# seungjunlee96/lightning-generative-models

Hardware: AMD Instinct MI355X
Metric: training images/sec (DDPM UNet 32x32, bs=128) (higher is better)
Workload: dtype f32

## Files before the change

lightning-generative-models_amd/csrc/winograd.hip:

```cpp
#include <stdlib.h>

#include <type_traits>

#include "lgm_common.h"

int lgm_splitk_reduce_launch(const float* ws, long ws_stride, int splits, const float* bias, const float* res,
                             long res_pitch, float* out, long out_pitch, long M, int N, hipStream_t s);

static void* lgm_wino_debug_buffer = nullptr;
static int lgm_wino_debug_mode = 0;
extern "C" int lgm_wino_set_debug_buffer(void* buf, int mode) {
  lgm_wino_debug_buffer = buf;
  lgm_wino_debug_mode = mode;
  return LGM_OK;
}

#ifndef LGM_STORE_AUX
#define LGM_STORE_AUX 0
#endif

namespace lgmwino {
typedef unsigned int u32x4 __attribute__((ext_vector_type(4)));
typedef float f32x2 __attribute__((ext_vector_type(2)));

// ... 1304 lines not shown
    w[k] = (double)gs[k]->B * gs[k]->H * gs[k]->W * gs[k]->Nw * gs[k]->Cw;
    tot += w[k];
    mn[k] = 2L * (gs[k]->Nw / 64) * (gs[k]->Cw / 32);
  }
  for (int k = 0; k < n; ++k) {
    long b = (long)((double)lgm_cu_budget() * w[k] / tot + (n == 2 && k == 0 ? 0.5 : 0.0));
    if (b < mn[k]) b = mn[k];
    budget[k] = b;
    left -= b;
  }
  int big = 0;
  for (int k = 1; k < n; ++k)
    if (budget[k] - mn[k] > budget[big] - mn[big]) big = k;
  budget[big] += left;
  if (budget[big] < mn[big]) budget[big] = mn[big];
}

static bool wgradn_supported(int n, const LgmConvGeom* const* gs) {
  using namespace lgmwino;
  if (n < 2 || n > 8) return false;
  if (n > 4) {
    for (int k = 0; k < n; ++k)
      if (!gs[k]) return false;
    return wgradn_use4(n, gs);
  }
  int G0 = 0;
  long need = 0;
  static const bool alone4 = getenv("LGM_W4W_ALONE") ? atoi(getenv("LGM_W4W_ALONE")) != 0 : true;
  if (alone4 && !wgradn_use4(n, gs)) {
    bool all4 = true;
    for (int k = 0; k < n; ++k) all4 = all4 && gs[k] && lgm_wino4_wgrad_use(gs[k]);
    if (all4) return false;
  }
  for (int k = 0; k < n; ++k) {
    if (!gs[k] || !lgm_wino_wgrad_supported(gs[k])) return false;
    int G, ipc;
    wgrad_class(gs[k]->H, gs[k]->W, &G, &ipc);
    if (k == 0) G0 = G;
    else if (G != G0) return false;
    need += 2L * (gs[k]->Nw / 64) * (gs[k]->Cw / 64);
  }
  return need <= lgm_cu_budget();
}

static void wgradn_budgets(int n, const LgmConvGeom* const* gs, long* budget) {
  double w[4], tot = 0;
  long mn[4], left = lgm_cu_budget();
  for (int k = 0; k < n; ++k) {
    w[k] = (double)gs[k]->B * gs[k]->H * gs[k]->W * gs[k]->Nw * gs[k]->Cw;
    tot += w[k];
    mn[k] = 2L * (gs[k]->Nw / 64) * (gs[k]->Cw / 64);
  }
  for (int k = 0; k < n; ++k) {
    long b = (long)((double)lgm_cu_budget() * w[k] / tot);
    if (b < mn[k]) b = mn[k];
    budget[k] = b;
    left -= b;
  }
  int big = 0;
  for (int k = 1; k < n; ++k)
    if (budget[k] - mn[k] > budget[big] - mn[big]) big = k;
  budget[big] += left;
  if (budget[big] < mn[big]) budget[big] = mn[big];
}

extern "C" int64_t lgm_conv3x3_wino_wgradn_supported(int n, const LgmConvGeom* const* geoms) {
// ... 280 lines not shown
```

lightning-generative-models_amd/csrc/winograd4.hip:

```cpp
#include <atomic>
#include <stdlib.h>

#include <type_traits>

#include "lgm_common.h"

int lgm_splitk_reduce_launch(const float* ws, long ws_stride, int splits, const float* bias, const float* res,
                             long res_pitch, float* out, long out_pitch, long M, int N, hipStream_t s);

static void* lgm_wino4_debug_buffer = nullptr;
static int lgm_wino4_debug_exp = 0;
static int lgm_wino4_debug_slots = 0;
static int lgm_wino4_debug_next = 0;
extern "C" int lgm_wino4_set_debug_buffer(void* buf, int exp) {
  lgm_wino4_debug_buffer = buf;
  lgm_wino4_debug_exp = exp & 0xffff;
  lgm_wino4_debug_slots = exp >> 16;
  lgm_wino4_debug_next = 0;
  return LGM_OK;
}

#ifndef LGM_WINO4_PFU
#define LGM_WINO4_PFU 1
#endif

namespace lgmwino4 {
typedef unsigned int u32x4 __attribute__((ext_vector_type(4)));
typedef float f32x2 __attribute__((ext_vector_type(2)));

constexpr int KC = 8;
constexpr int NXI = 36;
constexpr int VBUF = NXI * 256;
constexpr int MBUF = NXI * 32 * 32;

template <int CLS>
struct Geo;
template <>
struct Geo<0> {
  static constexpr int NI = 1, TTH = 4, TTW = 8, PH = 18, PW = 34, RS = 34, IMG = PH * RS, PLANE = 641;
};
template <>
struct Geo<1> {
  static constexpr int NI = 2, TTH = 4, TTW = 4, PH = 18, PW = 18, RS = 20, IMG = PH * RS, PLANE = 737;
};
template <>
struct Geo<2> {
  static constexpr int NI = 8, TTH = 2, TTW = 2, PH = 10, PW = 10, RS = 10, IMG = 112, PLANE = 897;
};

struct Args {
  const float* a;
  const float* u;
  const float* bias;
  const float* res;
  float* out;
  long a_pitch, res_pitch, out_pitch;
  int B, H, W;
  int C;
  int N;
  int tb_h, tb_w, tiles_n, nbg;
  int splits, pps, units;
  int tn_slowest;
  int xcd_ranges;
  float* ws;
  long ws_stride;
  long long* dbg;
  float* stats;
};

__device__ __forceinline__ f32x4 add4(const f32x4 a, const f32x4 b) { return a + b; }
__device__ __forceinline__ f32x4 sub4(const f32x4 a, const f32x4 b) {
  f32x2 lo, hi;
  asm("v_pk_add_f32 %0, %1, %2 neg_lo:[0,1] neg_hi:[0,1]"
      : "=v"(lo)
      : "v"(__builtin_shufflevector(a, a, 0, 1)), "v"(__builtin_shufflevector(b, b, 0, 1)));
  asm("v_pk_add_f32 %0, %1, %2 neg_lo:[0,1] neg_hi:[0,1]"
      : "=v"(hi)
      : "v"(__builtin_shufflevector(a, a, 2, 3)), "v"(__builtin_shufflevector(b, b, 2, 3)));
  return __builtin_shufflevector(lo, hi, 0, 1, 2, 3);
}
__device__ __forceinline__ f32x4 fma4(const float c, const f32x4 a, const f32x4 b) {
  return __builtin_elementwise_fma(f32x4{c, c, c, c}, a, b);
}
__device__ __forceinline__ f32x2 fma2(const float c, const f32x2 a, const f32x2 b) {
  return __builtin_elementwise_fma(f32x2{c, c}, a, b);
}

template <int CLS, bool DBG = false, int EXP = 0, bool STATS = false>
__global__ __launch_bounds__(512, 2) void wino4_conv_kernel(const Args p) {
  using GE = Geo<CLS>;
  constexpr bool PFU = LGM_WINO4_PFU != 0;
  int nstamp = 0;
  auto stamp = [&]() {
    if (DBG) {
      if (threadIdx.x == 0 && nstamp < 30) p.dbg[blockIdx.x * 32 + 1 + nstamp] = (long long)__builtin_amdgcn_s_memtime();
      ++nstamp;
    }
  };
  stamp();
  const long long rt_entry = DBG ? (long long)__builtin_amdgcn_s_memrealtime() : 0;
  constexpr int NI = GE::NI, PH = GE::PH, PW = GE::PW, RS = GE::RS, IMG = GE::IMG, PLANE = GE::PLANE;
  constexpr int RBUF = 8 * PLANE;
  constexpr int NPIX = NI * PH * PW;
  constexpr int NJ = (2 * NPIX + 511) / 512;
  extern __shared__ __align__(16) float smem[];
  float* const Rb = smem;
  float* const Vb = smem + 2 * RBUF;
  float* const Mb = smem;
  const int tid = threadIdx.x;
  const int lane = tid & 63;
  const int wid = __builtin_amdgcn_readfirstlane(tid >> 6);
  const int lr = lane & 31, lh = lane >> 5;

  int L = (p.xcd_ranges && (gridDim.x & 7) == 0) ? (int)((blockIdx.x & 7) * (gridDim.x >> 3) + (blockIdx.x >> 3)) : (int)blockIdx.x;
  int tn, split, twi, thi, bg;
  if (p.tn_slowest) {
    twi = L % p.tb_w;
    L /= p.tb_w;
    thi = L % p.tb_h;
    L /= p.tb_h;
    bg = L % p.nbg;
    L /= p.nbg;
    split = L % p.splits;
    tn = L / p.splits;
  } else {
    tn = L % p.tiles_n;
    L /= p.tiles_n;
    split = L % p.splits;
    L /= p.splits;
    twi = L % p.tb_w;
    L /= p.tb_w;
    thi = L % p.tb_h;
    bg = L / p.tb_h;
  }
  const int n0 = tn * 64;
  const int h0 = thi * (4 * GE::TTH), w0 = twi * (4 * GE::TTW), b0 = bg * NI;
  const int ncc = p.C / KC;
  const int cc0 = split * p.pps;
  const int cc1 = min(ncc, cc0 + p.pps);
  const int nph = cc1 - cc0;

  const unsigned nrec_a = (unsigned)((long)p.B * p.H * p.W * p.a_pitch * 4);
  __amdgpu_buffer_rsrc_t rsrc_a;
  {
    const unsigned long long ab = reinterpret_cast<unsigned long long>(p.a);
    const unsigned lo = __builtin_amdgcn_readfirstlane((unsigned)ab);
    const unsigned hi = __builtin_amdgcn_readfirstlane((unsigned)(ab >> 32));
    rsrc_a = __builtin_amdgcn_make_buffer_rsrc(reinterpret_cast<void*>(((unsigned long long)hi << 32) | lo), 0,
                                               __builtin_amdgcn_readfirstlane(nrec_a), 0x00020000);
  }
  unsigned goff[NJ], plds[NJ];
#pragma unroll
  for (int j = 0; j < NJ; ++j) {
    const int s = tid + 512 * j;
    const int pix = s >> 1, q = s & 1;
    unsigned g = nrec_a, l = (unsigned)(q * 4 * PLANE + NI * IMG);
    if (pix < NPIX) {
      const int img = pix / (PH * PW);
      const int rem = pix - img * (PH * PW);
      const int py = rem / PW, px = rem - py * PW;
      const int gy = h0 - 1 + py, gx = w0 - 1 + px;
      l = (unsigned)(q * 4 * PLANE + img * IMG + py * RS + px);
      if (gy >= 0 && gy < p.H && gx >= 0 && gx < p.W)
        g = (unsigned)((((long)(b0 + img) * p.H + gy) * p.W + gx) * p.a_pitch + q * 4) * 4u;
    }
    goff[j] = g;
    plds[j] = l;
  }
  u32x4 rp[NJ];
  auto fetch1 = [&](int j, int ph) -> u32x4 {
    const unsigned soff = (unsigned)((cc0 + ph) * (KC * 4));
    return __builtin_amdgcn_raw_buffer_load_b128(rsrc_a, ph < nph ? goff[j] : nrec_a, soff, 0);
  };
  auto commit_r = [&](float* rbuf, int j, const u32x4 r) {
    float* d = rbuf + plds[j];
    const f32x4 f = __builtin_bit_cast(f32x4, r);
    d[0] = f[0];
    d[PLANE] = f[1];
    d[2 * PLANE] = f[2];
    d[3 * PLANE] = f[3];
  };
  u32x4 rq0[NJ], rq1[NJ];
#pragma unroll
  for (int j = 0; j < NJ; ++j) rq0[j] = fetch1(j, 0);
#pragma unroll
  for (int j = 0; j < NJ; ++j) rq1[j] = fetch1(j, 1);
#pragma unroll
  for (int j = 0; j < NJ; ++j) rp[j] = fetch1(j, 2);

  int t_tile, t_img, t_ty, t_tx;
  const int half = wid >> 2;
  const int tk = (lane & 3) + 4 * (lane >> 5);
  if (CLS == 0) {
    t_img = 0;
    t_ty = wid & 3;
    t_tx = (lane >> 2) & 7;
    t_tile = t_ty * 8 + t_tx;
  } else if (CLS == 1) {
    t_img = (wid >> 1) & 1;
    t_ty = 2 * (wid & 1) + ((lane >> 4) & 1);
    t_tx = (lane >> 2) & 3;
    t_tile = t_img * 16 + t_ty * 4 + t_tx;
  } else {
    t_img = 2 * (wid & 3) + ((lane >> 4) & 1);
    t_ty = (lane >> 3) & 1;
    t_tx = (lane >> 2) & 1;
    t_tile = t_img * 4 + t_ty * 2 + t_tx;
  }
  const int trd = tk * PLANE + t_img * IMG + 4 * t_ty * RS + 4 * t_tx;
  const int vwr = (tk >> 2) * 128 + t_tile * 4 + (tk & 3) + half * (18 * 256);

  const int xg = wid & 3, ch = wid >> 2;
  const int vrd = xg * (9 * 256) + lh * 128 + lr * 4;
  __amdgpu_buffer_rsrc_t rsrc_u;
  {
    const unsigned long long ub = reinterpret_cast<unsigned long long>(p.u);
    const unsigned lo = __builtin_amdgcn_readfirstlane((unsigned)ub);
    const unsigned hi = __builtin_amdgcn_readfirstlane((unsigned)(ub >> 32));
    rsrc_u = __builtin_amdgcn_make_buffer_rsrc(reinterpret_cast<void*>(((unsigned long long)hi << 32) | lo), 0,
                                               __builtin_amdgcn_readfirstlane((unsigned)((long)p.N * p.C * NXI * 4)),
                                               0x00020000);
  }
  const unsigned ulane = (unsigned)((ch * 64 + lane) * 16);
  const unsigned ubase = (unsigned)((tn * ncc + cc0) * NXI + xg * 9) * 2048u;
  unsigned pf = 0;
  if (PFU) {
    const unsigned ubytes = min((unsigned)nph * (NXI * 2048u), 2u << 20);
    const unsigned nx = gridDim.x >> 3;
    const unsigned spatial = (unsigned)(p.nbg * p.tb_h * p.tb_w);
    const unsigned grp = p.tn_slowest ? 1u : (unsigned)(p.tiles_n * p.splits);
    const unsigned share = p.tn_slowest ? ((unsigned)blockIdx.x >> 3) % spatial : ((unsigned)blockIdx.x >> 3) / grp;
    const unsigned nshare = p.tn_slowest ? min(nx, spatial) : nx / grp;
    const unsigned off = (share * 512u + (unsigned)tid) * 128u;
    if (p.xcd_ranges && (gridDim.x & 7) == 0 && off < ubytes && nshare * 512u * 128u >= ubytes)
      pf = __builtin_amdgcn_raw_buffer_load_b32(rsrc_u, off, (unsigned)((tn * ncc + cc0) * NXI) * 2048u, 0);
  }
  auto load_u = [&](int ph, int e) -> f32x4 {
    const unsigned soff = ubase + (unsigned)(ph * NXI + e) * 2048u;
    u32x4 v = __builtin_amdgcn_raw_buffer_load_b128(rsrc_u, ulane, soff, 0);
    return __builtin_bit_cast(f32x4, v);
  };

  auto body = [&](auto half_c) {
    constexpr int HALF = decltype(half_c)::value;
    f32x16 acc[9];
#pragma unroll
    for (int e = 0; e < 9; ++e)
#pragma unroll
      for (int r = 0; r < 16; ++r) acc[e][r] = 0.f;
    f32x2 T[3][3];
    int roff0 = trd, roff1 = RBUF + trd;
    asm volatile("" : "+v"(roff0));
    asm volatile("" : "+v"(roff1));
    auto stage1 = [&](int nxt, int cp) {
      const float* r = smem + (nxt ? roff1 : roff0);
      f32x2 d[6];
#pragma unroll
      for (int rr = 0; rr < 6; ++rr)
        if (rr != (HALF ? 0 : 5)) d[rr] = f32x2{r[rr * RS + 2 * cp], r[rr * RS + 2 * cp + 1]};
      if (HALF == 0) {
        T[0][cp] = fma2(4.f, d[0], fma2(-5.f, d[2], d[4]));
        const f32x2 a = fma2(-4.f, d[2], d[4]), b = fma2(-4.f, d[1], d[3]);
        T[1][cp] = a + b;
        T[2][cp] = a - b;
      } else {
        const f32x2 c = d[4] - d[2], f = d[3] - d[1];
        T[0][cp] = fma2(2.f, f, c);
        T[1][cp] = fma2(-2.f, f, c);
        T[2][cp] = fma2(4.f, d[1], fma2(-5.f, d[3], d[5]));
      }
    };
    auto stage2 = [&](float* vbuf, int i, int part) {
      float* v = vbuf + vwr + i * (6 * 256);
      const float t0 = T[i][0][0], t1 = T[i][0][1], t2 = T[i][1][0], t3 = T[i][1][1], t4 = T[i][2][0], t5 = T[i][2][1];
      if (part == 0) {
        const float a = __builtin_fmaf(-4.f, t2, t4), b = __builtin_fmaf(-4.f, t1, t3);
        v[0 * 256] = __builtin_fmaf(4.f, t0, __builtin_fmaf(-5.f, t2, t4));
        v[1 * 256] = a + b;
        v[2 * 256] = a - b;
      } else {
        const float c = t4 - t2, f = t3 - t1;
        v[3 * 256] = __builtin_fmaf(2.f, f, c);
        v[4 * 256] = __builtin_fmaf(-2.f, f, c);
        v[5 * 256] = __builtin_fmaf(4.f, t1, __builtin_fmaf(-5.f, t3, t5));
      }
    };

    stamp();
    f32x4 uq[3];
#pragma unroll
    for (int e = 0; e < 3; ++e) uq[e] = load_u(0, e);
    if (DBG) __builtin_amdgcn_sched_barrier(0);
    stamp();
#pragma unroll
    for (int j = 0; j < NJ; ++j) commit_r(Rb, j, rq0[j]);
#pragma unroll
    for (int j = 0; j < NJ; ++j) commit_r(Rb + RBUF, j, rq1[j]);
    if (DBG) __builtin_amdgcn_sched_barrier(0);
    stamp();
    __syncthreads();
    if (PFU) asm volatile("" ::"v"(pf));
    stamp();
#pragma unroll
    for (int cp = 0; cp < 3; ++cp) stage1(0, cp);
#pragma unroll
    for (int i = 0; i < 3; ++i) {
      stage2(Vb, i, 0);
// ... 19 lines not shown
        for (int s = 0; s < 4; ++s) acc[e] = __builtin_amdgcn_mfma_f32_32x32x2f32(uf[s], vf[s], acc[e], 0, 0, 0);
        if (!(EXP & 4)) uq[e % 3] = (e + 3 < 9) ? load_u(ph, e + 3) : load_u(ph + 1, e + 3 - 9);
        if (!(EXP & 1)) {
          if (e < 3) stage1(cur ^ 1, e);
          else stage2(vnxt, (e - 3) >> 1, (e - 3) & 1);
        }
        if (e >= 9 - NJ && !(EXP & 2)) {
          commit_r(rcur, e - (9 - NJ), rp[e - (9 - NJ)]);
          rp[e - (9 - NJ)] = fetch1(e - (9 - NJ), ph + 3);
        }
        vf = vfn;
        __builtin_amdgcn_sched_barrier(0);
      }
      static_assert(NJ >= 1 && NJ <= 4, "the commit is dealt out over the last NJ steps");
      __syncthreads();
      stamp();
    };
    for (int ph = 0; ph < nph; ph += 2) {
      phase(ph, std::integral_constant<int, 0>{});
      if (ph + 1 < nph) phase(ph + 1, std::integral_constant<int, 1>{});
    }

    const int th = tid & 255;
    const int eq = th & 3, et = (th >> 2) & 31, rpair = __builtin_amdgcn_readfirstlane(th >> 7);
    int e_img, e_ty, e_tx;
    if (CLS == 0) {
      e_img = 0;
      e_ty = et >> 3;
      e_tx = et & 7;
    } else if (CLS == 1) {
      e_img = et >> 4;
      e_ty = (et >> 2) & 3;
      e_tx = et & 3;
    } else {
      e_img = et >> 2;
      e_ty = (et >> 1) & 1;
      e_tx = et & 1;
    }
    const long opix = ((long)(b0 + e_img) * p.H + h0 + 4 * e_ty) * p.W + w0 + 4 * e_tx;
    const bool partial = p.splits > 1;
    const int ncol0 = n0 + HALF * 16 + eq * 4;
    float* const obase = partial ? p.ws + (long)split * p.ws_stride + opix * p.N + ncol0 : p.out + opix * p.out_pitch + ncol0;
    const long opitch = partial ? (long)p.N : p.out_pitch;
    const bool has_res = !partial && p.res != nullptr;
    const float* const rbase = p.res + opix * p.res_pitch + ncol0;
    float* const Mh = Mb + HALF * (MBUF / 2);
    const int mrd = (et * 4 + (eq ^ ((et >> 1) & 3))) * 4;
    const int mwr = (lr * 4) * 4;
#pragma unroll
    for (int rd = 0; rd < 2; ++rd) {
      if (rd == 1) __syncthreads();
#pragma unroll
      for (int e = 0; e < 9; ++e)
#pragma unroll
        for (int gg = 0; gg < 2; ++gg) {
          const int g = 2 * rd + gg;
          const f32x4 v = {acc[e][4 * g], acc[e][4 * g + 1], acc[e][4 * g + 2], acc[e][4 * g + 3]};
          *reinterpret_cast<f32x4*>(Mh + (xg * 9 + e) * 512 + mwr + (((2 * gg + lh) ^ ((lr >> 1) & 3)) * 4)) = v;
        }
      __syncthreads();
      f32x4 X[2][6];
#pragma unroll
      for (int j = 0; j < 6; ++j) {
        auto m = [&](int i) -> f32x4 { return *reinterpret_cast<const f32x4*>(Mh + (i * 6 + j) * 512 + mrd); };
        const f32x4 m1 = m(1), m2 = m(2), m3 = m(3), m4 = m(4);
        if (rpair == 0) {
          const f32x4 s1 = add4(m1, m2), s2 = add4(m3, m4);
          X[0][j] = add4(add4(m(0), s1), s2);
          X[1][j] = fma4(4.f, s2, s1);
        } else {
// ... 122 lines not shown
    for (int s = 0; s < 4; ++s) {
      float g[9], u[36];
#pragma unroll
      for (int t = 0; t < 9; ++t) g[t] = wt[(n * 9 + t) * 36 + cq * 4 + s];
      ggt36(g, u);
#pragma unroll
      for (int x = 0; x < 36; ++x) uu[x][s] = u[x];
    }
    float* d = dst_f + row[3] + (((long)(nb >> 1) * (Cp / 8) + cb * 4 + (cq >> 1)) * NXI) * 512 +
               (((n >> 4) * 2 + (cq & 1)) * 32 + 16 * (nb & 1) + (n & 15)) * 4;
#pragma unroll
    for (int x = 0; x < 36; ++x) *reinterpret_cast<f32x4*>(d + x * 512) = uu[x];
  }
  if (dst_b) {
    const int c = tid & 31, nq = tid >> 5;
    f32x4 uu[36];
#pragma unroll
    for (int s = 0; s < 4; ++s) {
      float g[9], u[36];
#pragma unroll
      for (int t = 0; t < 9; ++t) g[8 - t] = wt[((nq * 4 + s) * 9 + t) * 36 + c];
      ggt36(g, u);
#pragma unroll
      for (int x = 0; x < 36; ++x) uu[x][s] = u[x];
    }
    float* d = dst_b + row[4] + (((long)(cb >> 1) * (Np / 8) + nb * 4 + (nq >> 1)) * NXI) * 512 +
               (((c >> 4) * 2 + (nq & 1)) * 32 + 16 * (cb & 1) + (c & 15)) * 4;
#pragma unroll
    for (int x = 0; x < 36; ++x) *reinterpret_cast<f32x4*>(d + x * 512) = uu[x];
  }
}

static long unit_count(int cls, int B, int H, int W) {
  return cls == 1 ? B / 2 : cls == 2 ? B / 8 : (long)B * (H / 16) * (W / 32);
}

static int unit_class(int H, int W) {
  if (H == 8 && W == 8) return 2;
  if (H == 16 && W == 16) return 1;
  if (H >= 16 && W >= 32 && H % 16 == 0 && W % 32 == 0) return 0;
  return -1;
}

}

bool lgm_wino4l_supported(const LgmConvGeom* g, int gather_channels, int out_channels);
long lgm_wino4l_units(const LgmConvGeom* g, int out_channels);
int lgm_wino4l_stats_parts(const LgmConvGeom* g);
int lgm_wino4l_class(const LgmConvGeom* g);
int lgm_wino4l_splits(const LgmConvGeom* g, int gather_channels, int out_channels);
int lgm_wino4l_launch(const LgmConvGeom* g, int yx, const float* a, long a_pitch, const float* u, const float* bias,
                      const float* res, long res_pitch, float* out, long out_pitch, void* workspace, long workspace_bytes,
                      hipStream_t s, int64_t* partial, float* stats);
static std::atomic<int> lgm_wino4_light_override{-1};
extern "C" int lgm_wino4_set_light(int mode) {
  lgm_wino4_light_override.store(mode, std::memory_order_relaxed);
  return LGM_OK;
}
static bool wino4_use_light(const LgmConvGeom* g, int gather_channels, int out_channels) {
  static const bool env_given = getenv("LGM_WINO4_LIGHT") != nullptr;
  static const int env_mode = env_given ? atoi(getenv("LGM_WINO4_LIGHT")) : 0;
  const int ov = lgm_wino4_light_override.load(std::memory_order_relaxed);
  const int mode = ov >= 0 ? ov : env_mode;
  if (!lgm_wino4l_supported(g, gather_channels, out_channels)) return false;
  if (mode != 0) return true;
  if (env_given || ov >= 0) return false;
  static long below[3] = {-1, 0, 0};
  if (below[0] < 0) {
    long b0 = 200, b1 = 128, b2 = 64;
    if (const char* e = getenv("LGM_WINO4_LIGHT_BELOW")) {
      b1 = b2 = -1;
      sscanf(e, "%ld,%ld,%ld", &b0, &b1, &b2);
      if (b1 < 0) b1 = b0;
      if (b2 < 0) b2 = b1;
    }
    below[1] = b1, below[2] = b2, below[0] = b0 < 0 ? 0 : b0;
  }
  const int cls = lgm_wino4l_class(g);
  return cls >= 0 && lgm_wino4l_units(g, out_channels) / 2 < below[cls];
}

static bool wino4_big_supported(const LgmConvGeom* g, int gather_channels, int out_channels);
bool lgm_wino4_supported(const LgmConvGeom* g, int gather_channels, int out_channels) {
  return wino4_use_light(g, gather_channels, out_channels) || wino4_big_supported(g, gather_channels, out_channels);
}
static bool wino4_big_supported(const LgmConvGeom* g, int gather_channels, int out_channels) {
  using namespace lgmwino4;
  if (!(g->KH == 3 && g->KW == 3 && g->stride == 1 && g->pad == 1)) return false;
  if (gather_channels % 8 != 0 || out_channels % 64 != 0 || gather_channels % 32 != 0) return false;
  const int cls = unit_class(g->H, g->W);
  if (cls < 0) return false;
  const long pix = (long)g->B * g->H * g->W + g->W + 1;
  if (pix * gather_channels >= (1L << 29) || pix * out_channels >= (1L << 29)) return false;
  if ((long)gather_channels * out_channels * 36 >= (1L << 29)) return false;
  return g->B % (cls == 1 ? 2 : cls == 2 ? 8 : 1) == 0;
}

int lgm_wino4_pick_splits(long base, long slots, int phases, int smax, int min_pps) {
  int s0 = (int)((slots + base - 1) / base);
  if (s0 > smax) s0 = smax;
  while (s0 > 1 && phases / s0 < min_pps) --s0;
  if (base * s0 <= slots) return s0;
  int best = s0;
  double best_cost = 1e30;
  for (int s = 1; s <= smax; ++s) {
    if (s > 1 && phases / s < min_pps) break;
    const long rounds = (base * s + slots - 1) / slots;
    const double pps = (double)((phases + s - 1) / s);
    const double cost = (double)rounds * (5.5 + pps) + (s > 1 ? 2.0 + 0.5 * s : 0.0);
    if (cost < best_cost - 1e-9) {
      best_cost = cost;
      best = s;
    }
  }
  return best;
}

int lgm_wino4_splits(const LgmConvGeom* g, int gather_channels, int out_channels) {
  using namespace lgmwino4;
  if (wino4_use_light(g, gather_channels, out_channels)) return lgm_wino4l_splits(g, gather_channels, out_channels);
  const int cls = unit_class(g->H, g->W);
  if (cls < 0) return 1;
  const long base = unit_count(cls, g->B, g->H, g->W) * (out_channels / 64);
  static const int forced = getenv("LGM_WINO4_SPLITS") ? atoi(getenv("LGM_WINO4_SPLITS")) : 0;
  const int phases = gather_channels / KC;
  int smax = phases / 2 < 16 ? phases / 2 : 16;
  if (smax < 1) smax = 1;
  if (forced > 0) return forced < smax ? forced : smax;
  const long slots = lgm_cu_budget();
  if (base >= slots * 3 / 4) return 1;
  static const int min_pps = getenv("LGM_WINO4_MIN_PPS") ? atoi(getenv("LGM_WINO4_MIN_PPS")) : 4;
  static const bool old_rule = getenv("LGM_WINO4_SPLITS_CEIL") != nullptr;
  if (old_rule) {
    int s = (int)((slots + base - 1) / base);
    if (s > smax) s = smax;
    while (s > 1 && phases / s < min_pps) --s;
    return s;
  }
  return lgm_wino4_pick_splits(base, slots, phases, smax, min_pps);
}

int lgm_wino4_launch(const LgmConvGeom* g, int yx, const float* a, long a_pitch, const float* u, const float* bias,
                     const float* res, long res_pitch, float* out, long out_pitch, void* workspace, long workspace_bytes,
                     hipStream_t s, int64_t* partial = nullptr, float* stats = nullptr) {
  using namespace lgmwino4;
  if (wino4_use_light(g, yx ? g->Nw : g->Cw, yx ? g->Cw : g->Nw))
    return lgm_wino4l_launch(g, yx, a, a_pitch, u, bias, res, res_pitch, out, out_pitch, workspace, workspace_bytes, s, partial,
                             stats);
  Args p{};
  p.stats = stats;
  p.a = a; p.u = u; p.bias = bias; p.res = res; p.out = out;
  p.a_pitch = a_pitch; p.res_pitch = res_pitch; p.out_pitch = out_pitch;
  p.B = g->B; p.H = g->H; p.W = g->W;
  p.C = yx ? g->Nw : g->Cw;
  p.N = yx ? g->Cw : g->Nw;
  const int cls = unit_class(g->H, g->W);
  p.tb_h = cls == 0 ? g->H / 16 : 1;
  p.tb_w = cls == 0 ? g->W / 32 : 1;
  p.nbg = cls == 1 ? g->B / 2 : cls == 2 ? g->B / 8 : g->B;
  p.tiles_n = p.N / 64;
  const long M = (long)g->B * g->H * g->W;
  p.splits = lgm_wino4_splits(g, p.C, p.N);
  if (p.splits > 1) {
    const long need = (long)p.splits * M * p.N * (long)sizeof(float);
    if (!workspace || workspace_bytes < need || !lgm_aligned16(workspace)) p.splits = 1;
  }
  p.ws = (float*)workspace;
  p.ws_stride = M * p.N;
  p.pps = lgm_cdiv(p.C / KC, p.splits);
  p.splits = lgm_cdiv(p.C / KC, p.pps);
  p.units = (int)((long)p.nbg * p.tb_h * p.tb_w * p.tiles_n * p.splits);
  {
    static const bool no_ranges = getenv("LGM_WINO4_NO_XCD_RANGES") != nullptr;
    p.xcd_ranges = no_ranges ? 0 : 1;
    static const int forced = getenv("LGM_WINO4_TN_SLOWEST") ? atoi(getenv("LGM_WINO4_TN_SLOWEST")) : -1;
    const double in_b = 1.2 * (double)M * p.C * 4.0, u_b = 36.0 * p.C * p.N * 4.0;
    p.tn_slowest = forced >= 0 ? forced : ((in_b + 8.0 * u_b > in_b * p.tiles_n + u_b) ? 1 : 0);
  }
  const size_t smem = (size_t)MBUF * sizeof(float);
  p.dbg = (long long*)lgm_wino4_debug_buffer;
  if (p.dbg && lgm_wino4_debug_slots > 0) {
    if (lgm_wino4_debug_next >= lgm_wino4_debug_slots || p.units > 4095) p.dbg = nullptr;
    else p.dbg += (long)(lgm_wino4_debug_next++) * 4096 * 32;
  }
#define LGM_W4LAUNCH(CC, DD, EE)                                                                                \
  do {                                                                                                          \
    auto kern = wino4_conv_kernel<CC, DD, EE>;                                                                        \
    static bool attr = false;                                                                                   \
    if (!attr) {                                                                                                \
      (void)hipFuncSetAttribute(reinterpret_cast<const void*>(kern), hipFuncAttributeMaxDynamicSharedMemorySize, \
                                (int)smem);                                                                     \
      attr = true;                                                                                              \
    }                                                                                                           \
    hipLaunchKernelGGL(kern, dim3((unsigned)p.units), dim3(512), smem, s, p);                                   \
  } while (0)
  lgm_note_kernel(cls == 0 ? LGM_KNAME("lgmwino4::wino4_conv_kernel<0, false, 0, false>") : cls == 1 ? LGM_KNAME("lgmwino4::wino4_conv_kernel<1, false, 0, false>")
                                                                                    : LGM_KNAME("lgmwino4::wino4_conv_kernel<2, false, 0, false>"));
  if (p.dbg) {
    const int e = lgm_wino4_debug_exp;
    if (cls == 1) LGM_W4LAUNCH(1, true, 0);
    else if (cls == 2) LGM_W4LAUNCH(2, true, 0);
    else if (e == 0) LGM_W4LAUNCH(0, true, 0);
    else if (e == 1) LGM_W4LAUNCH(0, true, 1);
    else if (e == 2) LGM_W4LAUNCH(0, true, 2);
    else if (e == 3) LGM_W4LAUNCH(0, true, 3);
    else if (e == 4) LGM_W4LAUNCH(0, true, 4);
    else if (e == 7) LGM_W4LAUNCH(0, true, 7);
    else if (e == 8) LGM_W4LAUNCH(0, true, 8);
    else LGM_W4LAUNCH(0, true, 15);
  } else if (stats) {
    if (cls != 0 || p.splits != 1 || res || partial) {
      lgm_set_error("wino4 (stats): class-0 maps, an unsplit reduction and no residual expected");
      return LGM_ERR_UNSUPPORTED;
    }
    auto kern = wino4_conv_kernel<0, false, 0, true>;
    static bool attr = false;
    if (!attr) {
      (void)hipFuncSetAttribute(reinterpret_cast<const void*>(kern), hipFuncAttributeMaxDynamicSharedMemorySize, (int)smem);
      attr = true;
    }
    lgm_note_kernel(LGM_KNAME("lgmwino4::wino4_conv_kernel<0, false, 0, true>"));
    hipLaunchKernelGGL(kern, dim3((unsigned)p.units), dim3(512), smem, s, p);
  } else if (cls == 0) LGM_W4LAUNCH(0, false, 0);
  else if (cls == 1) LGM_W4LAUNCH(1, false, 0);
  else LGM_W4LAUNCH(2, false, 0);
#undef LGM_W4LAUNCH
  if (partial) {
    partial[0] = p.splits;
    partial[1] = p.ws_stride;
    LGM_LAUNCH_CHECK();
    return LGM_OK;
  }
  if (p.splits > 1)
    return lgm_splitk_reduce_launch(p.ws, p.ws_stride, p.splits, bias, res, res_pitch, out, out_pitch, M, p.N, s);
  LGM_LAUNCH_CHECK();
  return LGM_OK;
}

extern "C" int64_t lgm_conv3x3_wino4_supported(const LgmConvGeom* g, int yx) {
  if (!g) return 0;
  return lgm_wino4_supported(g, yx ? g->Nw : g->Cw, yx ? g->Cw : g->Nw) ? 1 : 0;
}

extern "C" int64_t lgm_conv3x3_wino4_stats_floats(const LgmConvGeom* g, int* parts_per_image) {
  if (parts_per_image) *parts_per_image = 0;
  if (!g || !lgm_wino4_supported(g, g->Cw, g->Nw)) return 0;
  const bool light = wino4_use_light(g, g->Cw, g->Nw);
  if (light ? lgm_wino4l_stats_parts(g) == 0 : lgmwino4::unit_class(g->H, g->W) != 0) return 0;
  if (lgm_wino4_splits(g, g->Cw, g->Nw) != 1) return 0;
  static const bool off = getenv("LGM_NO_GN_EPI_STATS") != nullptr;
  if (off) return 0;
  const int per = light ? lgm_wino4l_stats_parts(g) : (g->H / 16) * (g->W / 32) * 4;
  if (parts_per_image) *parts_per_image = per;
  return (int64_t)g->B * per * 2 * g->Nw;
}

extern "C" int64_t lgm_conv3x3_wino4_workspace(const LgmConvGeom* g, int yx) {
  if (!g) return -1;
  const int gc = yx ? g->Nw : g->Cw, oc = yx ? g->Cw : g->Nw;
  if (!lgm_wino4_supported(g, gc, oc)) return 0;
  const int s = lgm_wino4_splits(g, gc, oc);
  return s > 1 ? (int64_t)s * g->B * g->H * g->W * oc * (int64_t)sizeof(float) : 0;
}

extern "C" int64_t lgm_conv3x3_wino4_preferred(const LgmConvGeom* g, int yx) {
  if (!g) return 0;
  const int gc = yx ? g->Nw : g->Cw, oc = yx ? g->Cw : g->Nw;
  if (!lgm_wino4_supported(g, gc, oc)) return 0;
  static const int force = getenv("LGM_WINO4_FORCE") ? atoi(getenv("LGM_WINO4_FORCE")) : 0;
  if (force) return 1;
  static const long min_units0_env = getenv("LGM_WINO4_MIN_UNITS") ? atol(getenv("LGM_WINO4_MIN_UNITS")) : -1;
  static const long min_units1_env = getenv("LGM_WINO4_MIN_UNITS1") ? atol(getenv("LGM_WINO4_MIN_UNITS1")) : -1;
  const long min_units0 = min_units0_env >= 0 ? min_units0_env : (wino4_use_light(g, gc, oc) ? 32 : 128);
  const long min_units1 = min_units1_env >= 0 ? min_units1_env : (wino4_use_light(g, gc, oc) ? 32 : 128);
  const bool light = wino4_use_light(g, gc, oc);
  const int cls = g->H == 8 && g->W == 8 ? 2 : g->H == 16 && g->W == 16 ? 1 : 0;
  const long base = light ? lgm_wino4l_units(g, oc) / 2 : lgmwino4::unit_count(cls, g->B, g->H, g->W) * (oc / 64);
  static const int fwd_all = getenv("LGM_WINO4_FWD_ALL") ? atoi(getenv("LGM_WINO4_FWD_ALL")) : 0;
  if (light && yx == 0 && fwd_all) return 1;
  static const int bwd_all = getenv("LGM_WINO4_BWD_ALL") ? atoi(getenv("LGM_WINO4_BWD_ALL")) : 0;
  if (light && yx == 1 && bwd_all) return 1;
  static const bool no8 = getenv("LGM_WINO4_NO8") != nullptr;
  static const bool noyx8 = getenv("LGM_WINO4_NOYX8") != nullptr;
  static const int c2_minc = getenv("LGM_WINO4_C2_MINC") ? atoi(getenv("LGM_WINO4_C2_MINC")) : 256;
  if (cls == 2) return (!no8 && (yx == 0 || !noyx8) && base >= 32 && gc >= c2_minc) ? 1 : 0;
  static const int c1_minc = getenv("LGM_WINO4_C1_MINC") ? atoi(getenv("LGM_WINO4_C1_MINC")) : 0;
  if (cls == 1 && gc < c1_minc) return 0;
  static const long min_units1w_env = getenv("LGM_WINO4_MIN_UNITS1W") ? atol(getenv("LGM_WINO4_MIN_UNITS1W")) : -1;
  const long min_units1w = min_units1w_env >= 0 ? min_units1w_env : (light ? 32 : 64);
  if (cls == 1 && gc >= 128 && base >= min_units1w) return 1;
  return base >= (cls == 1 ? min_units1 : min_units0) ? 1 : 0;
}

extern "C" int lgm_wino4_weights(const float* src, float* dst_f, float* dst_b, const int64_t* table, int n_slots,
                                 int64_t total_blocks, void* stream) {
  LGM_REQUIRE(src && table && n_slots > 0 && total_blocks > 0 && (dst_f || dst_b), "wino4_weights: bad arguments");
  hipLaunchKernelGGL(lgmwino4::wino4_weights_kernel, dim3((unsigned)total_blocks), dim3(256), 0, (hipStream_t)stream,
                     src, dst_f, dst_b, (const long*)table, n_slots);
  LGM_LAUNCH_CHECK();
  return LGM_OK;
}

extern "C" int lgm_conv3x3_wino4(int yx, const LgmConvGeom* g, const float* a, int64_t a_pitch, const float* u,
                                 const float* bias, const float* res, int64_t res_pitch, float* out, int64_t out_pitch,
                                 void* workspace, int64_t workspace_bytes, void* stream) {
  LGM_REQUIRE(g && a && u && out, "conv3x3_wino4: null pointer");
  const int gc = yx ? g->Nw : g->Cw, oc = yx ? g->Cw : g->Nw;
  LGM_REQUIRE(lgm_wino4_supported(g, gc, oc), "conv3x3_wino4: unsupported geometry (3x3/s1/p1, maps 16x16 or H %% 16 == 0 "
              "and W %% 32 == 0, reduction channels %% 32, produced channels %% 64)");
// ... 43 lines not shown
```

lightning-generative-models_amd/csrc/winograd4_wgrad.hip:

```cpp
#include <stdlib.h>

#include <type_traits>

#include "lgm_common.h"

#ifndef W4W_EXP
#define W4W_EXP 0
#endif

namespace lgmwino4w {
typedef unsigned int u32x4 __attribute__((ext_vector_type(4)));
typedef float f32x2 __attribute__((ext_vector_type(2)));

constexpr int NXI = 36;
constexpr int YB = NXI * 256;
constexpr int XB = NXI * 128;
constexpr int OPB = YB + XB;
constexpr int MH = NXI * 512;

struct WArgs {
  const float* y;
  const float* x;
  float* out;
  long y_pitch, x_pitch, slab;
// ... 52 lines not shown

  const unsigned nrec_y = (unsigned)((long)p.B * p.H * p.W * p.y_pitch * 4);
  const unsigned nrec_x = (unsigned)(((long)p.B * p.H * p.W + p.W + 1) * p.x_pitch * 4);
  auto rsrc = [&](const float* ptr, unsigned nrec) {
    const unsigned long long ab = reinterpret_cast<unsigned long long>(ptr);
    const unsigned lo = __builtin_amdgcn_readfirstlane((unsigned)ab);
    const unsigned hi = __builtin_amdgcn_readfirstlane((unsigned)(ab >> 32));
    return __builtin_amdgcn_make_buffer_rsrc(reinterpret_cast<void*>(((unsigned long long)hi << 32) | lo), 0,
                                             __builtin_amdgcn_readfirstlane(nrec), 0x00020000);
  };
  const __amdgpu_buffer_rsrc_t rsrc_y = rsrc(p.y, nrec_y);
  const __amdgpu_buffer_rsrc_t rsrc_x = rsrc(p.x - (long)(p.W + 1) * p.x_pitch, nrec_x);

  struct GPos {
    int gx, ty, b;
  };
  auto gdecode = [&](int g) {
    GPos q;
    q.gx = g % p.grow;
    const int r = g / p.grow;
    q.ty = r % p.trows;
    q.b = r / p.trows;
    return q;
  };
  auto gnext = [&](GPos& q) {
    if (++q.gx == p.grow) {
      q.gx = 0;
      if (++q.ty == p.trows) {
        q.ty = 0;
        ++q.b;
      }
    }
  };
  const int gh = p.sq ? 8 : 4, gw = p.sq ? 8 : 16;
  auto gpix = [&](const GPos& q) -> long { return ((long)q.b * p.H + gh * q.ty) * p.W + gw * q.gx; };
  auto tile_row = [&](int tl) { return p.sq ? (tl >> 1) : 0; };
  auto tile_col = [&](int tl) { return p.sq ? (tl & 1) : tl; };

  f32x16 acc[9];
#pragma unroll
  for (int e = 0; e < 9; ++e)
#pragma unroll
    for (int r = 0; r < 16; ++r) acc[e][r] = 0.f;

  auto mfma_step = [&](const float* buf, int e, f32x2& af, f32x2& bf) {
    f32x2 an = af, bn = bf;
    if (e < 8 && !(W4W_EXP & 8)) {
      an = *reinterpret_cast<const f32x2*>(buf + ard + (e + 1) * 256);
      bn = *reinterpret_cast<const f32x2*>(buf + brd + (e + 1) * 128);
    }
    acc[e] = __builtin_amdgcn_mfma_f32_32x32x2f32(af[0], bf[0], acc[e], 0, 0, 0);
    acc[e] = __builtin_amdgcn_mfma_f32_32x32x2f32(af[1], bf[1], acc[e], 0, 0, 0);
    af = an;
    bf = bn;
  };

  float bsum = 0.f;

  auto body_y = [&]() {
    const int tl = wid;
    const unsigned ylane = (unsigned)((((long)(4 * tile_row(tl)) * p.W + 4 * tile_col(tl)) * p.y_pitch + n0 + lane) * 4);
    const int ywr = (tl >> 1) * 128 + lane * 2 + (tl & 1);
    float dA[4][4], dB[4][4];
    GPos gq = gdecode(g_begin);
    auto load = [&](float (&d)[4][4], int ph) {
      const unsigned ok = ph < nph ? 0u : nrec_y;
      const unsigned ybase = (unsigned)(gpix(gq) * p.y_pitch * 4);
#pragma unroll
      for (int r = 0; r < 4; ++r)
#pragma unroll
        for (int c = 0; c < 4; ++c)
          d[r][c] = __builtin_bit_cast(float, __builtin_amdgcn_raw_buffer_load_b32(
              rsrc_y, ylane + ok, ybase + (unsigned)(((long)r * p.W + c) * p.y_pitch * 4), 0));
      if (ph + 1 < nph) gnext(gq);
    };
    float T[6][4];
    auto vertical2 = [&](const float (&d)[4][4], int cp) {
      const f32x2 d0 = {d[0][2 * cp], d[0][2 * cp + 1]}, d1 = {d[1][2 * cp], d[1][2 * cp + 1]};
      const f32x2 d2 = {d[2][2 * cp], d[2][2 * cp + 1]}, d3 = {d[3][2 * cp], d[3][2 * cp + 1]};
      const f32x2 s02 = d0 + d2, s13 = d1 + d3;
      const f32x2 e = fma2(4.f, d2, d0), f = fma2(4.f, d3, d1);
      const f32x2 t1 = s02 + s13, t2 = s02 - s13, t3 = fma2(2.f, f, e), t4 = fma2(-2.f, f, e);
#pragma unroll
      for (int k = 0; k < 2; ++k) {
        const int c = 2 * cp + k;
        T[0][c] = d0[k];
        T[1][c] = t1[k];
        T[2][c] = t2[k];
        T[3][c] = t3[k];
        T[4][c] = t4[k];
        T[5][c] = d3[k];
      }
      bsum += t1[0] + t1[1];
    };
// ... 22 lines not shown
      float* const onxt = smem + (cur ^ 1) * OPB;
      f32x2 af = *reinterpret_cast<const f32x2*>(ocur + ard);
      f32x2 bf = *reinterpret_cast<const f32x2*>(ocur + brd);
#pragma unroll
      for (int e = 0; e < 9; ++e) {
        mfma_step(ocur, e, af, bf);
        if (e == 0 && !(W4W_EXP & 4)) {
          if (cur == 0) load(dA, ph + 2);
          else load(dB, ph + 2);
        }
        if (e < 2) {
          if (!(W4W_EXP & 1)) {
            if (cur == 0) vertical2(dB, e);
            else vertical2(dA, e);
          }
        } else if (e < 8) {
          if (!(W4W_EXP & 1)) horizontal(onxt, e - 2);
        }
        __builtin_amdgcn_sched_barrier(0);
      }
      __syncthreads();
    };
    for (int ph = 0; ph < nph; ph += 2) {
      phase(ph, std::integral_constant<int, 0>{});
      if (ph + 1 < nph) phase(ph + 1, std::integral_constant<int, 1>{});
    }
  };

  auto body_x = [&](auto half_c) {
    constexpr int HALF = decltype(half_c)::value;
    const int tl = 2 * ((wid >> 1) & 1) + lh;
    const int c = lr;
    const int trow = tile_row(tl), tcol = tile_col(tl);
    const int tlast = p.sq ? 1 : 3;
    const unsigned xlane = (unsigned)((((long)(4 * trow) * p.W + 4 * tcol) * p.x_pitch + c0 + c) * 4);
    const int xwr = YB + (tl >> 1) * 64 + c * 2 + (tl & 1) + HALF * (18 * 128);
    constexpr int R0 = HALF ? 1 : 0;
    float d[5][6];
    GPos gq = gdecode(g_begin);
    auto load_rows = [&](int ph, int r_lo, int r_hi) {
      const GPos q = gq;
      const unsigned xbase = (unsigned)(gpix(q) * p.x_pitch * 4);
      const bool live = ph < nph;
#pragma unroll
      for (int r = 0; r < 5; ++r) {
        if (r < r_lo || r >= r_hi) continue;
        const int yy = gh * q.ty + 4 * trow - 1 + R0 + r;
        const bool rok = live && yy >= 0 && yy < p.H;
        const unsigned soff = rok ? xbase + (unsigned)((long)(R0 + r) * p.W * p.x_pitch * 4) : nrec_x;
#pragma unroll
        for (int cc = 0; cc < 6; ++cc) {
          unsigned vo = xlane + (unsigned)((long)cc * p.x_pitch * 4);
          if (cc == 0) vo = (q.gx == 0 && tcol == 0) ? nrec_x : vo;
          if (cc == 5) vo = (q.gx == p.grow - 1 && tcol == tlast) ? nrec_x : vo;
          d[r][cc] = __builtin_bit_cast(float, __builtin_amdgcn_raw_buffer_load_b32(rsrc_x, vo, soff, 0));
        }
      }
      if (r_hi == 5 && ph + 1 < nph) gnext(gq);
    };
    f32x2 T[3][3];
    auto stage1 = [&](int cp) {
      auto D = [&](int rr) { return f32x2{d[rr - R0][2 * cp], d[rr - R0][2 * cp + 1]}; };
      if (HALF == 0) {
        T[0][cp] = fma2(4.f, D(0), fma2(-5.f, D(2), D(4)));
        const f32x2 a = fma2(-4.f, D(2), D(4)), b = fma2(-4.f, D(1), D(3));
        T[1][cp] = a + b;
        T[2][cp] = a - b;
      } else {
// ... 123 lines not shown
__global__ __launch_bounds__(512, 2) void wino4_wgrad2_kernel(const WArgs pa, const WArgs pb, const int na) {
  if ((int)blockIdx.x < na) wino4_wgrad_body(pa, (int)blockIdx.x);
  else wino4_wgrad_body(pb, (int)blockIdx.x - na);
}

__global__ __launch_bounds__(512, 2) void wino4_wgrad4_kernel(const WArgs p0, const WArgs p1, const WArgs p2, const WArgs p3,
                                                               const int e0, const int e1, const int e2) {
  const int b = (int)blockIdx.x;
  if (b < e0) wino4_wgrad_body(p0, b);
  else if (b < e1) wino4_wgrad_body(p1, b - e0);
  else if (b < e2) wino4_wgrad_body(p2, b - e1);
  else wino4_wgrad_body(p3, b - e2);
}

struct WArgs8 {
  WArgs p[8];
  int e[7];
};
__global__ __launch_bounds__(512, 2) void wino4_wgrad8_kernel(const WArgs8 a) {
  const int b = (int)blockIdx.x;
  int k = 0;
#pragma unroll
  for (int i = 0; i < 7; ++i) k += b >= a.e[i] ? 1 : 0;
  const int base = k == 0 ? 0 : a.e[k - 1];
  wino4_wgrad_body(a.p[k], b - base);
}

}

bool lgm_wino4_wgrad_supported(const LgmConvGeom* g) {
  if (!(g->KH == 3 && g->KW == 3 && g->stride == 1 && g->pad == 1)) return false;
  if (g->Nw % 64 != 0 || g->Cw % 32 != 0) return false;
  const bool row_groups = g->W % 16 == 0 && g->H % 4 == 0, square_groups = g->W % 8 == 0 && g->H % 8 == 0;
  if (!row_groups && !square_groups) return false;
  const long groups = (long)g->B * g->H * g->W / 64;
  return groups >= 4;
}

extern "C" int64_t lgm_conv3x3_wino4_preferred(const LgmConvGeom* g, int yx);
bool lgm_wino4_wgrad_use(const LgmConvGeom* g) {
  static const bool off = getenv("LGM_NO_WINO4_WGRAD") != nullptr || getenv("LGM_NO_WINO4") != nullptr;
  return !off && lgm_wino4_wgrad_supported(g) && lgm_conv3x3_wino4_preferred(g, 1) != 0;
}

void lgm_wino4_wgrad_plan(const LgmConvGeom* g, long budget, int* splits, int* gps, int* total_groups) {
  const long groups = (long)g->B * g->H * g->W / 64;
  const long blocks = (long)(g->Nw / 64) * (g->Cw / 32);
  long smax = groups / 2 < budget ? groups / 2 : budget;
  if (smax < 2) smax = 2;
  long s = 2, best = -1;
  for (long c = 2; c <= smax; ++c) {
    const long rounds = (blocks * c + budget - 1) / budget;
    const long cost = rounds * ((groups + c - 1) / c + 6);
    if (best < 0 || cost < best) {
      best = cost;
      s = c;
    }
  }
  long per = (groups + s - 1) / s;
  s = (groups + per - 1) / per;
  *splits = (int)s;
  *gps = (int)per;
  *total_groups = (int)groups;
}

static void wino4_wgrad_prepare(const LgmConvGeom* g, const float* y, long y_pitch, const float* x, long x_pitch, float* out,
                                int bias, long slab, int splits, int gps, int total, lgmwino4w::WArgs& p) {
  p = lgmwino4w::WArgs{};
  p.y = y; p.x = x; p.out = out; p.bias = bias; p.slab = slab; p.y_pitch = y_pitch; p.x_pitch = x_pitch;
  p.B = g->B; p.H = g->H; p.W = g->W; p.Nw = g->Nw; p.Cw = g->Cw;
  p.tiles_c = g->Cw / 32;
  p.splits = splits; p.gps = gps; p.total_groups = total;
  p.sq = (g->W % 16 != 0) ? 1 : 0;
  static const int xcd_order = getenv("LGM_W4W_XCD") ? atoi(getenv("LGM_W4W_XCD")) : 1;
  p.xcd_order = xcd_order;
  p.grow = p.sq ? g->W / 8 : g->W / 16;
  p.trows = p.sq ? g->H / 8 : g->H / 4;
}

static constexpr size_t kW4Smem = (size_t)(2 * lgmwino4w::MH + 256) * sizeof(float);

int lgm_wino4_wgrad_launch(const LgmConvGeom* g, const float* y, long y_pitch, const float* x, long x_pitch, float* out,
                           int bias, long slab, int splits, int gps, int total, hipStream_t s) {
  using namespace lgmwino4w;
  WArgs p;
  wino4_wgrad_prepare(g, y, y_pitch, x, x_pitch, out, bias, slab, splits, gps, total, p);
  const unsigned nblocks = (unsigned)((g->Nw / 64) * (g->Cw / 32) * splits);
  static bool attr = false;
  if (!attr) {
    (void)hipFuncSetAttribute(reinterpret_cast<const void*>(wino4_wgrad_kernel), hipFuncAttributeMaxDynamicSharedMemorySize,
                              (int)kW4Smem);
    attr = true;
  }
  lgm_note_kernel(LGM_KNAME("lgmwino4w::wino4_wgrad_kernel"));
  hipLaunchKernelGGL(wino4_wgrad_kernel, dim3(nblocks), dim3(512), kW4Smem, s, p);
  LGM_LAUNCH_CHECK();
  return LGM_OK;
}

int lgm_wino4_wgradn_launch(int n, const LgmConvGeom* const* gs, const float* const* ys, const long* yps,
                            const float* const* xs, const long* xps, float* const* outs, const int* biases, const long* slabs,
                            const int* splits, const int* gpss, const int* totals, hipStream_t s) {
  using namespace lgmwino4w;
  WArgs pp[8];
  unsigned nb[8] = {0, 0, 0, 0, 0, 0, 0, 0};
  for (int k = 0; k < n; ++k) {
    wino4_wgrad_prepare(gs[k], ys[k], yps[k], xs[k], xps[k], outs[k], biases[k], slabs[k], splits[k], gpss[k], totals[k], pp[k]);
    nb[k] = (unsigned)((gs[k]->Nw / 64) * (gs[k]->Cw / 32) * splits[k]);
  }
  for (int k = n; k < 8; ++k) pp[k] = pp[n - 1];
// ... 76 lines not shown
```

Baseline: 13320.

## Extend F(4x4,3x3) Winograd conv and wgrad kernels to 4x4 feature maps

Adds a fourth tile class to the Winograd F(4,3) forward/dgrad kernel for 4x4 spatial inputs, packing 32 images per unit with no halo and specialized input transforms that skip the zero-padding rows and columns. It also extends the Winograd-4 weight-gradient kernel with an image-grouped mode (four 4x4 images per group) and routes the multi-conv wgrad path to it. The goal is to replace the slower fallback paths used for the smallest UNet resolution. The gain depends on enough channels and units, and the new transform code is a correctness risk.

```diff
diff --git a/lightning-generative-models_amd/csrc/winograd.hip b/lightning-generative-models_amd/csrc/winograd.hip
--- a/lightning-generative-models_amd/csrc/winograd.hip
+++ b/lightning-generative-models_amd/csrc/winograd.hip
@@ -1360,6 +1360,9 @@
     for (int k = 0; k < n; ++k) all4 = all4 && gs[k] && lgm_wino4_wgrad_use(gs[k]);
     if (all4) return false;
   }
+  if (wgradn_use4(n, gs))
+    for (int k = 0; k < n; ++k)
+      if (gs[k]->H == 4 && gs[k]->W == 4) return true;
   for (int k = 0; k < n; ++k) {
     if (!gs[k] || !lgm_wino_wgrad_supported(gs[k])) return false;
     int G, ipc;
diff --git a/lightning-generative-models_amd/csrc/winograd4.hip b/lightning-generative-models_amd/csrc/winograd4.hip
--- a/lightning-generative-models_amd/csrc/winograd4.hip
+++ b/lightning-generative-models_amd/csrc/winograd4.hip
@@ -46,6 +46,10 @@
 template <>
 struct Geo<2> {
   static constexpr int NI = 8, TTH = 2, TTW = 2, PH = 10, PW = 10, RS = 10, IMG = 112, PLANE = 897;
+};
+template <>
+struct Geo<3> {
+  static constexpr int NI = 32, TTH = 1, TTW = 1, PH = 4, PW = 4, RS = 4, IMG = 20, PLANE = 641;
 };
 
 struct Args {
@@ -103,6 +107,7 @@
   constexpr int RBUF = 8 * PLANE;
   constexpr int NPIX = NI * PH * PW;
   constexpr int NJ = (2 * NPIX + 511) / 512;
+  constexpr int HALO = CLS == 3 ? 0 : 1;
   extern __shared__ __align__(16) float smem[];
   float* const Rb = smem;
   float* const Vb = smem + 2 * RBUF;
@@ -159,7 +164,7 @@
       const int img = pix / (PH * PW);
       const int rem = pix - img * (PH * PW);
       const int py = rem / PW, px = rem - py * PW;
-      const int gy = h0 - 1 + py, gx = w0 - 1 + px;
+      const int gy = h0 - HALO + py, gx = w0 - HALO + px;
       l = (unsigned)(q * 4 * PLANE + img * IMG + py * RS + px);
       if (gy >= 0 && gy < p.H && gx >= 0 && gx < p.W)
         g = (unsigned)((((long)(b0 + img) * p.H + gy) * p.W + gx) * p.a_pitch + q * 4) * 4u;
@@ -201,11 +206,16 @@
     t_ty = 2 * (wid & 1) + ((lane >> 4) & 1);
     t_tx = (lane >> 2) & 3;
     t_tile = t_img * 16 + t_ty * 4 + t_tx;
-  } else {
+  } else if (CLS == 2) {
     t_img = 2 * (wid & 3) + ((lane >> 4) & 1);
     t_ty = (lane >> 3) & 1;
     t_tx = (lane >> 2) & 1;
     t_tile = t_img * 4 + t_ty * 2 + t_tx;
+  } else {
+    t_img = 8 * (wid & 3) + ((lane >> 2) & 7);
+    t_ty = 0;
+    t_tx = 0;
+    t_tile = t_img;
   }
   const int trd = tk * PLANE + t_img * IMG + 4 * t_ty * RS + 4 * t_tx;
   const int vwr = (tk >> 2) * 128 + t_tile * 4 + (tk & 3) + half * (18 * 256);
@@ -254,6 +264,26 @@
     asm volatile("" : "+v"(roff1));
     auto stage1 = [&](int nxt, int cp) {
       const float* r = smem + (nxt ? roff1 : roff0);
+      if constexpr (CLS == 3) {
+        f32x2 d[5];
+#pragma unroll
+        for (int rr = 1; rr < 5; ++rr) {
+          const float* q = r + (rr - 1) * RS;
+          d[rr] = cp == 0 ? f32x2{0.f, q[0]} : cp == 1 ? f32x2{q[1], q[2]} : f32x2{q[3], 0.f};
+        }
+        if (HALF == 0) {
+          T[0][cp] = fma2(-5.f, d[2], d[4]);
+          const f32x2 a = fma2(-4.f, d[2], d[4]), b = fma2(-4.f, d[1], d[3]);
+          T[1][cp] = a + b;
+          T[2][cp] = a - b;
+        } else {
+          const f32x2 c = d[4] - d[2], f = d[3] - d[1];
+          T[0][cp] = fma2(2.f, f, c);
+          T[1][cp] = fma2(-2.f, f, c);
+          T[2][cp] = fma2(4.f, d[1], d[3] * -5.f);
+        }
+        return;
+      }
       f32x2 d[6];
 #pragma unroll
       for (int rr = 0; rr < 6; ++rr)
@@ -273,6 +303,20 @@
     auto stage2 = [&](float* vbuf, int i, int part) {
       float* v = vbuf + vwr + i * (6 * 256);
       const float t0 = T[i][0][0], t1 = T[i][0][1], t2 = T[i][1][0], t3 = T[i][1][1], t4 = T[i][2][0], t5 = T[i][2][1];
+      if constexpr (CLS == 3) {
+        if (part == 0) {
+          const float a = __builtin_fmaf(-4.f, t2, t4), b = __builtin_fmaf(-4.f, t1, t3);
+          v[0 * 256] = __builtin_fmaf(-5.f, t2, t4);
+          v[1 * 256] = a + b;
+          v[2 * 256] = a - b;
+        } else {
+          const float c = t4 - t2, f = t3 - t1;
+          v[3 * 256] = __builtin_fmaf(2.f, f, c);
+          v[4 * 256] = __builtin_fmaf(-2.f, f, c);
+          v[5 * 256] = __builtin_fmaf(4.f, t1, t3 * -5.f);
+        }
+        return;
+      }
       if (part == 0) {
         const float a = __builtin_fmaf(-4.f, t2, t4), b = __builtin_fmaf(-4.f, t1, t3);
         v[0 * 256] = __builtin_fmaf(4.f, t0, __builtin_fmaf(-5.f, t2, t4));
@@ -358,10 +402,14 @@
       e_img = et >> 4;
       e_ty = (et >> 2) & 3;
       e_tx = et & 3;
-    } else {
+    } else if (CLS == 2) {
       e_img = et >> 2;
       e_ty = (et >> 1) & 1;
       e_tx = et & 1;
+    } else {
+      e_img = et;
+      e_ty = 0;
+      e_tx = 0;
     }
     const long opix = ((long)(b0 + e_img) * p.H + h0 + 4 * e_ty) * p.W + w0 + 4 * e_tx;
     const bool partial = p.splits > 1;
@@ -550,10 +598,11 @@
 }
 
 static long unit_count(int cls, int B, int H, int W) {
-  return cls == 1 ? B / 2 : cls == 2 ? B / 8 : (long)B * (H / 16) * (W / 32);
+  return cls == 1 ? B / 2 : cls == 2 ? B / 8 : cls == 3 ? B / 32 : (long)B * (H / 16) * (W / 32);
 }
 
 static int unit_class(int H, int W) {
+  if (H == 4 && W == 4) return 3;
   if (H == 8 && W == 8) return 2;
   if (H == 16 && W == 16) return 1;
   if (H >= 16 && W >= 32 && H % 16 == 0 && W % 32 == 0) return 0;
@@ -574,6 +623,12 @@
 extern "C" int lgm_wino4_set_light(int mode) {
   lgm_wino4_light_override.store(mode, std::memory_order_relaxed);
   return LGM_OK;
+}
+static bool wino4_light_asked() {
+  static const bool env_given = getenv("LGM_WINO4_LIGHT") != nullptr;
+  static const int env_mode = env_given ? atoi(getenv("LGM_WINO4_LIGHT")) : 0;
+  const int ov = lgm_wino4_light_override.load(std::memory_order_relaxed);
+  return (ov >= 0 ? ov : env_mode) != 0;
 }
 static bool wino4_use_light(const LgmConvGeom* g, int gather_channels, int out_channels) {
   static const bool env_given = getenv("LGM_WINO4_LIGHT") != nullptr;
@@ -611,7 +666,7 @@
   const long pix = (long)g->B * g->H * g->W + g->W + 1;
   if (pix * gather_channels >= (1L << 29) || pix * out_channels >= (1L << 29)) return false;
   if ((long)gather_channels * out_channels * 36 >= (1L << 29)) return false;
-  return g->B % (cls == 1 ? 2 : cls == 2 ? 8 : 1) == 0;
+  return g->B % (cls == 1 ? 2 : cls == 2 ? 8 : cls == 3 ? 32 : 1) == 0;
 }
 
 int lgm_wino4_pick_splits(long base, long slots, int phases, int smax, int min_pps) {
@@ -675,7 +730,7 @@
   const int cls = unit_class(g->H, g->W);
   p.tb_h = cls == 0 ? g->H / 16 : 1;
   p.tb_w = cls == 0 ? g->W / 32 : 1;
-  p.nbg = cls == 1 ? g->B / 2 : cls == 2 ? g->B / 8 : g->B;
+  p.nbg = cls == 1 ? g->B / 2 : cls == 2 ? g->B / 8 : cls == 3 ? g->B / 32 : g->B;
   p.tiles_n = p.N / 64;
   const long M = (long)g->B * g->H * g->W;
   p.splits = lgm_wino4_splits(g, p.C, p.N);
@@ -713,11 +768,12 @@
     hipLaunchKernelGGL(kern, dim3((unsigned)p.units), dim3(512), smem, s, p);                                   \
   } while (0)
   lgm_note_kernel(cls == 0 ? LGM_KNAME("lgmwino4::wino4_conv_kernel<0, false, 0, false>") : cls == 1 ? LGM_KNAME("lgmwino4::wino4_conv_kernel<1, false, 0, false>")
-                                                                                    : LGM_KNAME("lgmwino4::wino4_conv_kernel<2, false, 0, false>"));
+                  : cls == 2 ? LGM_KNAME("lgmwino4::wino4_conv_kernel<2, false, 0, false>") : LGM_KNAME("lgmwino4::wino4_conv_kernel<3, false, 0, false>"));
   if (p.dbg) {
     const int e = lgm_wino4_debug_exp;
     if (cls == 1) LGM_W4LAUNCH(1, true, 0);
     else if (cls == 2) LGM_W4LAUNCH(2, true, 0);
+    else if (cls == 3) LGM_W4LAUNCH(3, true, 0);
     else if (e == 0) LGM_W4LAUNCH(0, true, 0);
     else if (e == 1) LGM_W4LAUNCH(0, true, 1);
     else if (e == 2) LGM_W4LAUNCH(0, true, 2);
@@ -741,7 +797,8 @@
     hipLaunchKernelGGL(kern, dim3((unsigned)p.units), dim3(512), smem, s, p);
   } else if (cls == 0) LGM_W4LAUNCH(0, false, 0);
   else if (cls == 1) LGM_W4LAUNCH(1, false, 0);
-  else LGM_W4LAUNCH(2, false, 0);
+  else if (cls == 2) LGM_W4LAUNCH(2, false, 0);
+  else LGM_W4LAUNCH(3, false, 0);
 #undef LGM_W4LAUNCH
   if (partial) {
     partial[0] = p.splits;
@@ -792,7 +849,13 @@
   const long min_units0 = min_units0_env >= 0 ? min_units0_env : (wino4_use_light(g, gc, oc) ? 32 : 128);
   const long min_units1 = min_units1_env >= 0 ? min_units1_env : (wino4_use_light(g, gc, oc) ? 32 : 128);
   const bool light = wino4_use_light(g, gc, oc);
-  const int cls = g->H == 8 && g->W == 8 ? 2 : g->H == 16 && g->W == 16 ? 1 : 0;
+  const int cls = g->H == 4 && g->W == 4 ? 3 : g->H == 8 && g->W == 8 ? 2 : g->H == 16 && g->W == 16 ? 1 : 0;
+  if (cls == 3) {
+    static const bool no4 = getenv("LGM_WINO4_NO4") != nullptr;
+    const int narrow = gc < oc ? gc : oc;
+    const long units = lgmwino4::unit_count(3, g->B, g->H, g->W) * (narrow / 64);
+    return (!no4 && !wino4_light_asked() && narrow >= 256 && units >= 32) ? 1 : 0;
+  }
   const long base = light ? lgm_wino4l_units(g, oc) / 2 : lgmwino4::unit_count(cls, g->B, g->H, g->W) * (oc / 64);
   static const int fwd_all = getenv("LGM_WINO4_FWD_ALL") ? atoi(getenv("LGM_WINO4_FWD_ALL")) : 0;
   if (light && yx == 0 && fwd_all) return 1;
diff --git a/lightning-generative-models_amd/csrc/winograd4_wgrad.hip b/lightning-generative-models_amd/csrc/winograd4_wgrad.hip
--- a/lightning-generative-models_amd/csrc/winograd4_wgrad.hip
+++ b/lightning-generative-models_amd/csrc/winograd4_wgrad.hip
@@ -108,10 +108,13 @@
       }
     }
   };
-  const int gh = p.sq ? 8 : 4, gw = p.sq ? 8 : 16;
-  auto gpix = [&](const GPos& q) -> long { return ((long)q.b * p.H + gh * q.ty) * p.W + gw * q.gx; };
-  auto tile_row = [&](int tl) { return p.sq ? (tl >> 1) : 0; };
-  auto tile_col = [&](int tl) { return p.sq ? (tl & 1) : tl; };
+  const int gh = p.sq == 1 ? 8 : 4, gw = p.sq == 1 ? 8 : p.sq == 2 ? 4 : 16;
+  auto gpix = [&](const GPos& q) -> long {
+    return ((long)(p.sq == 2 ? 4 * q.b : q.b) * p.H + gh * q.ty) * p.W + gw * q.gx;
+  };
+  auto tile_row = [&](int tl) { return p.sq == 1 ? (tl >> 1) : 0; };
+  auto tile_col = [&](int tl) { return p.sq == 1 ? (tl & 1) : p.sq == 2 ? 0 : tl; };
+  auto tile_img = [&](int tl) { return p.sq == 2 ? tl : 0; };
 
   f32x16 acc[9];
 #pragma unroll
@@ -135,7 +138,8 @@
 
   auto body_y = [&]() {
     const int tl = wid;
-    const unsigned ylane = (unsigned)((((long)(4 * tile_row(tl)) * p.W + 4 * tile_col(tl)) * p.y_pitch + n0 + lane) * 4);
+    const unsigned ylane =
+        (unsigned)(((((long)tile_img(tl) * p.H + 4 * tile_row(tl)) * p.W + 4 * tile_col(tl)) * p.y_pitch + n0 + lane) * 4);
     const int ywr = (tl >> 1) * 128 + lane * 2 + (tl & 1);
     float dA[4][4], dB[4][4];
     GPos gq = gdecode(g_begin);
@@ -224,8 +228,9 @@
     const int tl = 2 * ((wid >> 1) & 1) + lh;
     const int c = lr;
     const int trow = tile_row(tl), tcol = tile_col(tl);
-    const int tlast = p.sq ? 1 : 3;
-    const unsigned xlane = (unsigned)((((long)(4 * trow) * p.W + 4 * tcol) * p.x_pitch + c0 + c) * 4);
+    const int tlast = p.sq == 1 ? 1 : p.sq == 2 ? 0 : 3;
+    const unsigned xlane =
+        (unsigned)(((((long)tile_img(tl) * p.H + 4 * trow) * p.W + 4 * tcol) * p.x_pitch + c0 + c) * 4);
     const int xwr = YB + (tl >> 1) * 64 + c * 2 + (tl & 1) + HALF * (18 * 128);
     constexpr int R0 = HALF ? 1 : 0;
     float d[5][6];
@@ -415,7 +420,8 @@
   if (!(g->KH == 3 && g->KW == 3 && g->stride == 1 && g->pad == 1)) return false;
   if (g->Nw % 64 != 0 || g->Cw % 32 != 0) return false;
   const bool row_groups = g->W % 16 == 0 && g->H % 4 == 0, square_groups = g->W % 8 == 0 && g->H % 8 == 0;
-  if (!row_groups && !square_groups) return false;
+  const bool image_groups = g->H == 4 && g->W == 4 && g->B % 4 == 0;
+  if (!row_groups && !square_groups && !image_groups) return false;
   const long groups = (long)g->B * g->H * g->W / 64;
   return groups >= 4;
 }
@@ -454,11 +460,11 @@
   p.B = g->B; p.H = g->H; p.W = g->W; p.Nw = g->Nw; p.Cw = g->Cw;
   p.tiles_c = g->Cw / 32;
   p.splits = splits; p.gps = gps; p.total_groups = total;
-  p.sq = (g->W % 16 != 0) ? 1 : 0;
+  p.sq = (g->H == 4 && g->W == 4) ? 2 : (g->W % 16 != 0) ? 1 : 0;
   static const int xcd_order = getenv("LGM_W4W_XCD") ? atoi(getenv("LGM_W4W_XCD")) : 1;
   p.xcd_order = xcd_order;
-  p.grow = p.sq ? g->W / 8 : g->W / 16;
-  p.trows = p.sq ? g->H / 8 : g->H / 4;
+  p.grow = p.sq == 2 ? 1 : p.sq ? g->W / 8 : g->W / 16;
+  p.trows = p.sq == 2 ? 1 : p.sq ? g->H / 8 : g->H / 4;
 }
 
 static constexpr size_t kW4Smem = (size_t)(2 * lgmwino4w::MH + 256) * sizeof(float);
```

Measured after the change: 13580, median of 6. 2.0% higher.
